# BVE-Reborn/rend3

Hardware: NVIDIA H100
Metric: culled objects/s (fused frustum cull + object-uniform bake) (higher is better)
Workload: dtype f32

## Files before the change

rend3_b200/csrc/r3_cull_bake.cu:

```cuda
#include <cstdlib>

#include "r3_common.cuh"
#include "r3_scan.cuh"

namespace {

constexpr int CB_THREADS = 256;
constexpr int CB_WARPS = CB_THREADS / 32;
constexpr int CB_WT = 4;
constexpr int CB_CTA_OBJECTS = CB_WARPS * CB_WT * 32;
constexpr int CP_THREADS = 1024;
constexpr int CP_OBJECTS = CP_THREADS * 32;
constexpr int CP_CTAS_PER_TILE = CP_OBJECTS / CB_CTA_OBJECTS;

struct CullBakeParams {
    float view[16];
    float view_proj[16];
    float frustum[5][4];
    uint32_t object_count;
};

__device__ __forceinline__ uint32_t affine_w_bits(uint32_t j) { return j == 3 ? 0x3f800000u : 0u; }

__global__ void __launch_bounds__(256) split_objects_kernel(const float4* __restrict__ objects, uint32_t n, float* __restrict__ rows_xyz, float* __restrict__ rows_w,
                                                            float4* __restrict__ spheres, uint32_t* __restrict__ enabled_bits, uint32_t* __restrict__ affine_bits) {
    const int lane = threadIdx.x & 31, k = lane & 7, g = lane >> 3;
    const uint32_t wtile = (blockIdx.x * blockDim.x + threadIdx.x) >> 5, base = wtile * 32u;
    if (base >= n) return;
    uint32_t bits = 0, abits = 0;
#pragma unroll
    for (int it = 0; it < 8; ++it) {
        const uint32_t obj = base + it * 4 + g;
        float4 r = make_float4(0.f, 0.f, 0.f, 0.f);
        if (obj < n) {
            r = __ldcs(&objects[(size_t)obj * 8 + k]);
            if (k < 4) {
                float* xyz = rows_xyz + (size_t)obj * 12 + k;
                xyz[0] = r.x; xyz[4] = r.y; xyz[8] = r.z;
                rows_w[(size_t)obj * 4 + k] = r.w;
            } else if (k == 4) spheres[obj] = r;
        }
        const uint32_t b = __ballot_sync(0xFFFFFFFFu, k == 7 && obj < n && __float_as_uint(r.y) != 0u);
        bits |= (((b >> 7) & 1u) | (((b >> 15) & 1u) << 1) | (((b >> 23) & 1u) << 2) | (((b >> 31) & 1u) << 3)) << (it * 4);
        const uint32_t a = __ballot_sync(0xFFFFFFFFu, k < 4 && obj < n && __float_as_uint(r.w) == affine_w_bits(k));
#pragma unroll
        for (int q = 0; q < 4; ++q) abits |= (((a >> (8 * q)) & 0xFu) == 0xFu ? 1u : 0u) << (it * 4 + q);
    }
    if (lane == 0) { enabled_bits[wtile] = bits; affine_bits[wtile] = abits; }
}
__global__ void __launch_bounds__(256) split_slots_kernel(const float4* __restrict__ objects, const uint32_t* __restrict__ slots, uint32_t n_updates, uint32_t n_slots,
                                                          float* __restrict__ rows_xyz, float* __restrict__ rows_w, float4* __restrict__ spheres,
                                                          uint32_t* __restrict__ enabled_bits, uint32_t* __restrict__ affine_bits) {
    const uint32_t i = (blockIdx.x * blockDim.x + threadIdx.x) >> 3, k = threadIdx.x & 7;
    const uint32_t s = i < n_updates ? slots[i] : n_slots;
    const bool ok = s < n_slots;
    float4 r = make_float4(0.f, 0.f, 0.f, 0.f);
    if (ok) {
        r = objects[(size_t)s * 8 + k];
        if (k < 4) {
            float* xyz = rows_xyz + (size_t)s * 12 + k;
            xyz[0] = r.x; xyz[4] = r.y; xyz[8] = r.z;
            rows_w[(size_t)s * 4 + k] = r.w;
        } else if (k == 4) spheres[s] = r;
    }
    const uint32_t a = __ballot_sync(0xFFFFFFFFu, ok && k < 4 && __float_as_uint(r.w) == affine_w_bits(k));
    if (ok && k == 7) {
        const uint32_t bit = 1u << (s & 31u);
        if (__float_as_uint(r.y) != 0u) atomicOr(&enabled_bits[s >> 5], bit);
        else atomicAnd(&enabled_bits[s >> 5], ~bit);
        if (((a >> (threadIdx.x & 24u)) & 0xFu) == 0xFu) atomicOr(&affine_bits[s >> 5], bit);
        else atomicAnd(&affine_bits[s >> 5], ~bit);
    }
}

template <bool BAKE, bool CULL, bool LIVE>
__global__ void __launch_bounds__(CB_THREADS)
cull_bake_kernel(const float4* __restrict__ rows_xyz, const float* __restrict__ rows_w, const uint32_t* __restrict__ affine_bits, const float4* __restrict__ spheres,
                 const uint32_t* __restrict__ enabled_bits, const uint32_t* __restrict__ live_bits, float4* __restrict__ matrices, uint32_t* __restrict__ words,
                 uint32_t* __restrict__ cta_counts, const __grid_constant__ CullBakeParams p) {
    __shared__ uint32_t s_count[CB_WARPS];
    __shared__ float4 s_rows[BAKE ? CB_WARPS : 1][96];
    const int lane = threadIdx.x & 31, warp = threadIdx.x >> 5;
    const int col = lane & 3, sub = lane >> 2;
    uint32_t count = 0;
#pragma unroll 2
    for (int wt = 0; wt < CB_WT; ++wt) {
        const uint32_t wtile = (blockIdx.x * CB_WARPS + warp) * CB_WT + wt;
        const uint32_t base = wtile * 32u;
        if (base >= p.object_count) break;
        float4 t[3];
        float4 sp = make_float4(0.f, 0.f, 0.f, 0.f);
        uint32_t enabled = 0u, affine = 0u;
        if (BAKE) {
#pragma unroll
            for (int q = 0; q < 3; ++q) {
                const uint32_t e = q * 32 + lane;
                t[q] = base + e / 3u < p.object_count ? __ldcs(&rows_xyz[(size_t)base * 3 + e]) : make_float4(0.f, 0.f, 0.f, 0.f);
            }
        }
        if (CULL && base + lane < p.object_count) sp = __ldcs(&spheres[base + lane]);
        if (BAKE || (CULL && !LIVE)) enabled = __ldg(&enabled_bits[wtile]);
        if (BAKE) affine = __ldg(&affine_bits[wtile]);
        if (BAKE) {
            float4* tile = s_rows[warp];
            __syncwarp();
#pragma unroll
            for (int q = 0; q < 3; ++q) tile[q * 32 + lane] = t[q];
            __syncwarp();
            const float* tf = reinterpret_cast<const float*>(tile);
#pragma unroll
            for (int it = 0; it < 4; ++it) {
                const uint32_t slot = it * 8 + sub, obj = base + slot;
                if (obj < p.object_count && ((enabled >> slot) & 1u)) {
                    const float* c = tf + slot * 12 + col;
                    const float w = ((affine >> slot) & 1u) ? (col == 3 ? 1.0f : 0.0f) : __ldcs(&rows_w[(size_t)obj * 4 + col]);
                    float4* dst = &matrices[(size_t)obj * 8 + col];
                    __stcs(dst, mat_vec_rn(p.view, c[0], c[4], c[8], w));
                    __stcs(dst + 4, mat_vec_rn(p.view_proj, c[0], c[4], c[8], w));
                }
            }
        }
        if (CULL) {
            const uint32_t live = LIVE ? __ldg(&live_bits[wtile]) : enabled;
            const float neg_radius = -sp.w;
            bool inside = true;
#pragma unroll
            for (int pl = 0; pl < 5; ++pl) {
                const float d = add_rn(add_rn(add_rn(mul_rn(p.frustum[pl][0], sp.x), mul_rn(p.frustum[pl][1], sp.y)), mul_rn(p.frustum[pl][2], sp.z)), p.frustum[pl][3]);
                inside = inside && (d >= neg_radius);
            }
            const uint32_t word = __ballot_sync(0xFFFFFFFFu, base + lane < p.object_count && ((live >> lane) & 1u) && inside);
            if (lane == 0) words[wtile] = word;
            count += __popc(word);
        }
    }
    if (CULL) {
        if (lane == 0) s_count[warp] = count;
        __syncthreads();
        if (threadIdx.x == 0) {
            uint32_t t = 0;
#pragma unroll
            for (int w = 0; w < CB_WARPS; ++w) t += s_count[w];
            cta_counts[blockIdx.x] = t;
        }
    }
}

constexpr uint32_t EX_HEADER_WORDS = 256;
constexpr uint32_t EX_SLOTS = R3_EXCHANGE_SLOTS;
struct ExchangeParams { uint32_t* peers[R3_MAX_EXCHANGE_RANKS]; uint32_t n_ranks, word_offset, words_per_rank, flag_offset, epoch; uint32_t* done; };

__device__ __forceinline__ void st_release_sys(uint32_t* p, uint32_t v) { asm volatile("st.release.sys.global.u32 [%0], %1;" ::"l"(p), "r"(v) : "memory"); }
__device__ __forceinline__ uint32_t ld_acquire_sys(const uint32_t* p) { uint32_t v; asm volatile("ld.acquire.sys.global.u32 %0, [%1];" : "=r"(v) : "l"(p) : "memory"); return v; }

__global__ void __launch_bounds__(CP_THREADS)
compact_visible_kernel(const uint32_t* __restrict__ words, const uint32_t* __restrict__ cta_counts, uint32_t n_words, uint32_t n_cta_counts,
                       uint32_t* __restrict__ visible, uint32_t* __restrict__ visible_count, const __grid_constant__ ExchangeParams ex) {
    __shared__ uint32_t s_warp[CP_THREADS / 32 + 1];
    const uint32_t tile_base = block_sum_u32<CP_THREADS>(cta_counts, min(blockIdx.x * CP_CTAS_PER_TILE, n_cta_counts), s_warp);
    const uint32_t wi = blockIdx.x * CP_THREADS + threadIdx.x;
    const uint32_t word = wi < n_words ? __ldg(&words[wi]) : 0u;
    if (ex.n_ranks && wi < ex.words_per_rank) {
// ... 403 lines not shown
```

rend3_b200/csrc/r3_raster.cu:

```cuda
#include "r3_common.cuh"
#include "r3_scan.cuh"
#include "r3_texture.cuh"

namespace {

constexpr int RS_THREADS = 256;
constexpr float GUARD = 64.0f;
constexpr int SMALL_AREA = 64;
constexpr int MEDIUM_MAX = 32;
constexpr int COOP_MAX_LANES = 33;
constexpr int BAND_ROWS = 16;
constexpr uint32_t LARGE_CAP = 1u << 22;
constexpr uint32_t BAND_CAP = 1u << 24;
constexpr uint32_t BAND_SKIP = 0xFFFFFFFFu;
constexpr int MODE_COLOUR = 0;
constexpr int MODE_DEPTH = 1;
constexpr int MODE_BLEND = 2;
constexpr int MODE_MSAA = 4;
constexpr int MODE_ALPHA = 8;

struct SubTri { int32_t x[3], y[3]; float z[3]; uint32_t rec; };
constexpr uint32_t REC_ALPHA_TESTED = 0x80000000u;
static_assert(sizeof(SubTri) == 40, "SubTri");

struct RasterParams {
    const r3_batch_data* batches; const r3_region* regions; const uint32_t* header;
    const r3_indirect_call* calls; const uint32_t* indices; uint64_t index_elems;
    const unsigned long long* tri_prefix;
    const r3_object* objects; uint32_t n_slots;
    const r3_object_matrices* matrices; uint32_t matrices_cap;
    const uint32_t* mesh; uint64_t mesh_words;
    const r3_material* materials; uint32_t n_materials;
    TexTable tt;
    float ox, oy, vw, vh; int32_t x0, y0, x1, y1; uint32_t pitch; int positive_visible;
    uint32_t samples;
    unsigned long long* vis; uint32_t pass_bit;
    uint32_t* depth_bits;
    r3_tri_record* records;
    SubTri* large; uint2* bands; uint32_t* counters;
    uint32_t* frag_heads; uint4* frag_nodes; uint32_t frag_cap;
    unsigned long long key_lo, key_hi;
    unsigned long long* stats;
};

__device__ __forceinline__ uint32_t mesh_word(const RasterParams& p, uint64_t i) { return i < p.mesh_words ? __ldg(&p.mesh[i]) : 0u; }

__device__ __forceinline__ float plane_dist(int plane, const float4 v) {
    switch (plane) {
        case 0: return v.z;
        case 1: return sub_rn(v.w, v.z);
        case 2: return add_rn(v.x, mul_rn(GUARD, v.w));
        case 3: return sub_rn(mul_rn(GUARD, v.w), v.x);
        case 4: return add_rn(v.y, mul_rn(GUARD, v.w));
        default: return sub_rn(mul_rn(GUARD, v.w), v.y);
    }
}
__device__ __forceinline__ float4 clip_lerp(const float4 in, const float4 out, float din, float dout) {
    const float t = div_rn(din, sub_rn(din, dout));
    return make_float4(add_rn(in.x, mul_rn(t, sub_rn(out.x, in.x))), add_rn(in.y, mul_rn(t, sub_rn(out.y, in.y))),
                       add_rn(in.z, mul_rn(t, sub_rn(out.z, in.z))), add_rn(in.w, mul_rn(t, sub_rn(out.w, in.w))));
}
__device__ __noinline__ int clip_polygon(float4* poly, int n) {
    for (int plane = 0; plane < 6 && n >= 3; ++plane) {
        bool any_out = false;
        for (int i = 0; i < n; ++i) any_out |= plane_dist(plane, poly[i]) < 0.0f;
        if (!any_out) continue;
        float4 outp[12];
        int m = 0;
        for (int i = 0; i < n; ++i) {
            const float4 a = poly[i], b = poly[(i + 1) % n];
            const float da = plane_dist(plane, a), db = plane_dist(plane, b);
            if (da >= 0.0f) {
                outp[m++] = a;
                if (db < 0.0f) outp[m++] = clip_lerp(a, b, da, db);
            } else if (db >= 0.0f) {
                outp[m++] = clip_lerp(b, a, db, da);
            }
        }
        n = m;
        for (int i = 0; i < n; ++i) poly[i] = outp[i];
    }
    return n >= 3 ? n : 0;
}

constexpr int FITS32_REACH = 11585;
template <typename T>
struct EdgeSetupT {
    T e0, e1, e2;
    T sx0, sx1, sx2;
    T sy0, sy1, sy2;
    int b0, b1, b2;
    float inv_area;
};
__device__ __forceinline__ float to_float_rn(long long v) { return __ll2float_rn(v); }
__device__ __forceinline__ float to_float_rn(int v) { return __int2float_rn(v); }
__device__ __forceinline__ long long edge_fn(int ax, int ay, int bx, int by, long long px, long long py) {
    return (long long)(bx - ax) * (py - ay) - (long long)(by - ay) * (px - ax);
}
__device__ __forceinline__ int not_top_left(int ax, int ay, int bx, int by) {
    const int dx = bx - ax, dy = by - ay;
    return ((dy < 0) || (dy == 0 && dx > 0)) ? 0 : 1;
}
__device__ __forceinline__ bool fits32(const SubTri& s, int px0, int py0, int px1, int py1) {
    const int ox = px0 * 256 + 128, oy = py0 * 256 + 128;
    int reach = max((px1 - px0) * 256 + 128, (py1 - py0) * 256 + 128);
#pragma unroll
    for (int k = 0; k < 3; ++k) reach = max(reach, max(abs(s.x[k] - ox), abs(s.y[k] - oy)));
    return reach <= FITS32_REACH && abs(px0) < (1 << 20) && abs(py0) < (1 << 20);
}
template <typename T>
__device__ __forceinline__ EdgeSetupT<T> make_edges(const SubTri& s, int px, int py) {
    EdgeSetupT<T> e;
    e.b0 = not_top_left(s.x[1], s.y[1], s.x[2], s.y[2]);
    e.b1 = not_top_left(s.x[2], s.y[2], s.x[0], s.y[0]);
    e.b2 = not_top_left(s.x[0], s.y[0], s.x[1], s.y[1]);
    const int ox = px * 256 + 128, oy = py * 256 + 128;
    const T x0 = (T)s.x[0] - ox, y0 = (T)s.y[0] - oy, x1 = (T)s.x[1] - ox, y1 = (T)s.y[1] - oy, x2 = (T)s.x[2] - ox, y2 = (T)s.y[2] - oy;
    e.e0 = (x2 - x1) * (-y1) - (y2 - y1) * (-x1) - e.b0;
    e.e1 = (x0 - x2) * (-y2) - (y0 - y2) * (-x2) - e.b1;
    e.e2 = (x1 - x0) * (-y0) - (y1 - y0) * (-x0) - e.b2;
    e.sx0 = -(y2 - y1) * 256; e.sy0 = (x2 - x1) * 256;
    e.sx1 = -(y0 - y2) * 256; e.sy1 = (x0 - x2) * 256;
    e.sx2 = -(y1 - y0) * 256; e.sy2 = (x1 - x0) * 256;
    const T area = (x1 - x0) * (y2 - y0) - (y1 - y0) * (x2 - x0);
    e.inv_area = div_rn(1.0f, to_float_rn(area));
    return e;
}
template <typename T>
__device__ __forceinline__ float sample_depth(const SubTri& s, const EdgeSetupT<T>& e, T e0, T e1, T e2) {
    const float la = mul_rn(to_float_rn((T)(e0 + e.b0)), e.inv_area), lb = mul_rn(to_float_rn((T)(e1 + e.b1)), e.inv_area),
                lc = mul_rn(to_float_rn((T)(e2 + e.b2)), e.inv_area);
    const float z = add_rn(add_rn(mul_rn(la, s.z[0]), mul_rn(lb, s.z[1])), mul_rn(lc, s.z[2]));
    return fminf(fmaxf(z, 0.0f), 1.0f);
}
template <int MODE>
__device__ __forceinline__ uint32_t write_sample(const RasterParams& p, int px, int py, uint32_t k, float z, uint32_t rec) {
    const size_t pi = (size_t)py * p.pitch + px;
    if ((MODE & 3) == MODE_DEPTH) {
        atomicMax(&p.depth_bits[pi], __float_as_uint(z));
    } else if ((MODE & 3) == MODE_COLOUR) {
        const unsigned long long key = ((unsigned long long)__float_as_uint(z) << 32) | ((unsigned long long)p.pass_bit << 31) | (rec & ~REC_ALPHA_TESTED);
        atomicMax(&p.vis[pi * p.samples + k], key);
    } else {
        const size_t si = pi * p.samples + k;
        if (__float_as_uint(z) >= (uint32_t)(p.vis[si] >> 32)) {
            const uint32_t node = atomicAdd(&p.counters[3], 1u);
            if (node < p.frag_cap) {
                const uint32_t next = atomicExch(&p.frag_heads[si], node + 1u);
                p.frag_nodes[node] = make_uint4(rec & ~REC_ALPHA_TESTED, __float_as_uint(z), next, 0u);
            }
        }
        return 0u;
    }
    return 1u;
}

__device__ __constant__ int c_sample_dx[4] = {-32, 96, -96, 32};
__device__ __constant__ int c_sample_dy[4] = {-96, -32, 32, 96};

template <int MODE>
__device__ __noinline__ bool cutout_discards(const RasterParams& p, uint32_t rec, int px, int py) {
    const r3_tri_record* tp = p.records + ((rec & ~REC_ALPHA_TESTED) - 1u);
    const float4 q0 = reinterpret_cast<const float4*>(tp)[0], q1 = reinterpret_cast<const float4*>(tp)[1], q2 = reinterpret_cast<const float4*>(tp)[2];
    const uint4 q3 = reinterpret_cast<const uint4*>(tp)[3];
    const float p0[3] = {q0.x, q0.y, q0.z}, p1[3] = {q0.w, q1.x, q1.y}, p2[3] = {q1.z, q1.w, q2.x};
    const uint32_t oid = __float_as_uint(q2.y);
    const uint32_t vid[3] = {__float_as_uint(q2.z), __float_as_uint(q2.w), q3.x};
    const r3_object* obj = &p.objects[oid];
    const r3_material* m = &p.materials[obj->material_index < p.n_materials ? obj->material_index : 0u];
    const uint32_t flags = m->flags;
    float alpha = 1.0f;
    if (flags & R3_MAT_ALBEDO_ACTIVE) {
        const float hw = p.vw * 0.5f, hh = p.vh * 0.5f;
        float b[3][3];
#pragma unroll
        for (int k = 0; k < 3; ++k) {
            const float fx = ((float)px - p.ox) + (k == 1 ? 1.5f : 0.5f), fy = ((float)py - p.oy) + (k == 2 ? 1.5f : 0.5f);
            const float nx = fx / hw - 1.0f, ny = 1.0f - fy / hh;
            const float b0 = ((p1[1] * p2[2] - p1[2] * p2[1]) * nx + (p1[2] * p2[0] - p1[0] * p2[2]) * ny) + (p1[0] * p2[1] - p1[1] * p2[0]);
            const float b1 = ((p2[1] * p0[2] - p2[2] * p0[1]) * nx + (p2[2] * p0[0] - p2[0] * p0[2]) * ny) + (p2[0] * p0[1] - p2[1] * p0[0]);
            const float b2 = ((p0[1] * p1[2] - p0[2] * p1[1]) * nx + (p0[2] * p1[0] - p0[0] * p1[2]) * ny) + (p0[0] * p1[1] - p0[1] * p1[0]);
            const float sum = (b0 + b1) + b2;
            b[k][0] = b0 / sum; b[k][1] = b1 / sum; b[k][2] = b2 / sum;
        }
        const uint32_t albedo_tex = m->textures[R3_TEX_ALBEDO];
        if (albedo_tex) {
            float uv[3][2] = {{0.f, 0.f}, {0.f, 0.f}, {0.f, 0.f}};
            const uint32_t uv_off = obj->attr_offset[3];
            if (uv_off != R3_ATTR_ABSENT) {
#pragma unroll
                for (int k = 0; k < 3; ++k) {
                    const uint64_t w = (uint64_t)(uv_off >> 2) + (uint64_t)vid[k] * 2u;
                    uv[k][0] = __uint_as_float(mesh_word(p, w)); uv[k][1] = __uint_as_float(mesh_word(p, w + 1));
                }
            }
            float co[3][2];
#pragma unroll
            for (int k = 0; k < 3; ++k) {
                const float u = (b[k][0] * uv[0][0] + b[k][1] * uv[1][0]) + b[k][2] * uv[2][0];
                const float v = (b[k][0] * uv[0][1] + b[k][1] * uv[1][1]) + b[k][2] * uv[2][1];
                if ((MODE & 3) == MODE_DEPTH) { co[k][0] = u; co[k][1] = v; }
                else {
                    co[k][0] = (m->uv_transform0[0][0] * u + m->uv_transform0[1][0] * v) + m->uv_transform0[2][0];
                    co[k][1] = (m->uv_transform0[0][1] * u + m->uv_transform0[1][1] * v) + m->uv_transform0[2][1];
                }
            }
            TexCoords tc;
            tc.u = co[0][0]; tc.v = co[0][1];
            tc.dudx = co[1][0] - co[0][0]; tc.dvdx = co[1][1] - co[0][1];
            if ((MODE & 3) == MODE_DEPTH) { tc.dudy = tc.dudx; tc.dvdy = tc.dvdx; }
            else { tc.dudy = co[2][0] - co[0][0]; tc.dvdy = co[2][1] - co[0][1]; }
            alpha = texture_sample_grad(p.tt, albedo_tex, (MODE & 3) != MODE_DEPTH && (flags & R3_MAT_NEAREST), tc).w;
        }
        if (flags & R3_MAT_ALBEDO_BLEND) {
            float va[3] = {1.0f, 1.0f, 1.0f};
            const uint32_t col_off = obj->attr_offset[5];
            if (col_off != R3_ATTR_ABSENT) {
#pragma unroll
                for (int k = 0; k < 3; ++k) va[k] = (float)(mesh_word(p, (uint64_t)(col_off >> 2) + vid[k]) >> 24) / 255.0f;
            }
            alpha *= (b[0][0] * va[0] + b[0][1] * va[1]) + b[0][2] * va[2];
        }
    }
    return alpha * m->albedo[3] < m->alpha_cutout;
}

template <int MODE, typename T>
__device__ __forceinline__ void emit_pixel(const RasterParams& p, const SubTri& s, const EdgeSetupT<T>& e, int px, int py, T c0, T c1, T c2, uint32_t& frags) {
    if (!(MODE & MODE_MSAA)) {
        if ((c0 | c1 | c2) >= 0) {
            if ((MODE & MODE_ALPHA) && (s.rec & REC_ALPHA_TESTED) && cutout_discards<MODE>(p, s.rec, px, py)) return;
            frags += write_sample<MODE>(p, px, py, 0u, sample_depth<T>(s, e, c0, c1, c2), s.rec);
        }
        return;
    }
    bool tested = !(MODE & MODE_ALPHA) || !(s.rec & REC_ALPHA_TESTED);
#pragma unroll
    for (int k = 0; k < 4; ++k) {
        const T a0 = c0 + (e.sx0 >> 8) * c_sample_dx[k] + (e.sy0 >> 8) * c_sample_dy[k];
        const T a1 = c1 + (e.sx1 >> 8) * c_sample_dx[k] + (e.sy1 >> 8) * c_sample_dy[k];
        const T a2 = c2 + (e.sx2 >> 8) * c_sample_dx[k] + (e.sy2 >> 8) * c_sample_dy[k];
        if ((a0 | a1 | a2) >= 0) {
            if (!tested) {
                if (cutout_discards<MODE>(p, s.rec, px, py)) return;
                tested = true;
            }
            frags += write_sample<MODE>(p, px, py, (uint32_t)k, sample_depth<T>(s, e, a0, a1, a2), s.rec);
        }
    }
}

__device__ __forceinline__ void pixel_bounds(const RasterParams& p, const SubTri& s, int& px0, int& py0, int& px1, int& py1) {
    const int minx = min(s.x[0], min(s.x[1], s.x[2])), maxx = max(s.x[0], max(s.x[1], s.x[2]));
    const int miny = min(s.y[0], min(s.y[1], s.y[2])), maxy = max(s.y[0], max(s.y[1], s.y[2]));
    if (p.samples == 1u) {
        px0 = max((minx - 128 + 255) >> 8, p.x0); px1 = min((maxx - 128) >> 8, p.x1 - 1);
        py0 = max((miny - 128 + 255) >> 8, p.y0); py1 = min((maxy - 128) >> 8, p.y1 - 1);
    } else {
        px0 = max(minx >> 8, p.x0); px1 = min(maxx >> 8, p.x1 - 1);
        py0 = max(miny >> 8, p.y0); py1 = min(maxy >> 8, p.y1 - 1);
    }
}

template <int MODE, typename T>
__device__ __forceinline__ void raster_inline_t(const RasterParams& p, const SubTri& s, int px0, int py0, int px1, int py1, uint32_t& frags) {
    const EdgeSetupT<T> e = make_edges<T>(s, px0, py0);
    T r0 = e.e0, r1 = e.e1, r2 = e.e2;
    for (int py = py0; py <= py1; ++py) {
        T c0 = r0, c1 = r1, c2 = r2;
        for (int px = px0; px <= px1; ++px) {
            emit_pixel<MODE, T>(p, s, e, px, py, c0, c1, c2, frags);
            c0 += e.sx0; c1 += e.sx1; c2 += e.sx2;
        }
        r0 += e.sy0; r1 += e.sy1; r2 += e.sy2;
    }
}
template <int MODE>
__device__ __forceinline__ void raster_inline(const RasterParams& p, const SubTri& s, int px0, int py0, int px1, int py1, uint32_t& frags) {
    if (fits32(s, px0, py0, px1, py1)) raster_inline_t<MODE, int>(p, s, px0, py0, px1, py1, frags);
    else raster_inline_t<MODE, long long>(p, s, px0, py0, px1, py1, frags);
}

template <int MODE>
__device__ bool process_subtriangle(const RasterParams& p, const float4 a, const float4 b, const float4 c, uint32_t rec, uint32_t& frags, SubTri* defer,
                                    bool* deferred) {
    const float4 v[3] = {a, b, c};
    int sx[3], sy[3];
    float sz[3];
    const float hw = mul_rn(p.vw, 0.5f), hh = mul_rn(p.vh, 0.5f);
#pragma unroll
    for (int k = 0; k < 3; ++k) {
        if (!(v[k].w > 0.0f)) return false;
        const bool unit_w = v[k].w == 1.0f;
        const float nx = unit_w ? v[k].x : div_rn(v[k].x, v[k].w), ny = unit_w ? v[k].y : div_rn(v[k].y, v[k].w), nz = unit_w ? v[k].z : div_rn(v[k].z, v[k].w);
        const float fx = add_rn(p.ox, mul_rn(add_rn(nx, 1.0f), hw)), fy = add_rn(p.oy, mul_rn(sub_rn(1.0f, ny), hh));
        const float qx = rintf(mul_rn(fx, 256.0f)), qy = rintf(mul_rn(fy, 256.0f));
        if (!(fabsf(qx) < 1.0e9f) || !(fabsf(qy) < 1.0e9f)) return false;
        sx[k] = (int)qx; sy[k] = (int)qy; sz[k] = nz;
    }
    const long long area = (long long)(sx[1] - sx[0]) * (sy[2] - sy[0]) - (long long)(sx[2] - sx[0]) * (sy[1] - sy[0]);
    if (area == 0) return false;
    const bool visible = p.positive_visible ? (area < 0) : (area > 0);
    if (!visible) return false;
    SubTri s;
    if (area > 0) {
#pragma unroll
        for (int k = 0; k < 3; ++k) { s.x[k] = sx[k]; s.y[k] = sy[k]; s.z[k] = sz[k]; }
    } else {
        s.x[0] = sx[0]; s.y[0] = sy[0]; s.z[0] = sz[0]; s.x[1] = sx[2]; s.y[1] = sy[2]; s.z[1] = sz[2]; s.x[2] = sx[1]; s.y[2] = sy[1]; s.z[2] = sz[1];
    }
    s.rec = rec;
    int px0, py0, px1, py1;
    pixel_bounds(p, s, px0, py0, px1, py1);
    if (px0 > px1 || py0 > py1) return true;
    const int w = px1 - px0 + 1, h = py1 - py0 + 1;
    bool inline_raster = (w * h <= SMALL_AREA);
    if (!inline_raster && defer && w <= MEDIUM_MAX && h <= MEDIUM_MAX) {
        *defer = s;
        *deferred = true;
        return true;
    }
    if (!inline_raster) {
        const uint32_t nb = (uint32_t)((py1 / BAND_ROWS) - (py0 / BAND_ROWS) + 1);
        const uint32_t li = atomicAdd(&p.counters[0], 1u);
        uint32_t bi = 0;
        bool queued = li < LARGE_CAP;
        if (queued) {
            bi = atomicAdd(&p.counters[1], nb);
            queued = bi + nb <= BAND_CAP;
            if (!queued) for (uint32_t k = bi; k < BAND_CAP; ++k) p.bands[k] = make_uint2(BAND_SKIP, 0u);
        }
        if (queued) {
            p.large[li] = s;
            for (uint32_t k = 0; k < nb; ++k) p.bands[bi + k] = make_uint2(li, (uint32_t)(py0 / BAND_ROWS) + k);
            return true;
        }
        if (defer) {
            *defer = s;
            *deferred = true;
            return true;
        }
        inline_raster = true;
    }
    raster_inline<MODE>(p, s, px0, py0, px1, py1, frags);
    return true;
}

template <int MODE, typename T>
__device__ __forceinline__ void raster_cooperative_t(const RasterParams& p, const SubTri& s, int lane, int px0, int py0, int px1, int py1, uint32_t& frags) {
    const int w = px1 - px0 + 1;
    const int lw = w <= 8 ? 8 : (w <= 16 ? 16 : 32), lh = 32 / lw, lx = lane % lw, ly = lane / lw;
    const EdgeSetupT<T> e = make_edges<T>(s, px0, py0);
    for (int py = py0 + ly; py <= py1; py += lh) {
        const T dy = py - py0;
        T c0 = e.e0 + dy * e.sy0 + (T)lx * e.sx0, c1 = e.e1 + dy * e.sy1 + (T)lx * e.sx1, c2 = e.e2 + dy * e.sy2 + (T)lx * e.sx2;
        for (int px = px0 + lx; px <= px1; px += lw) {
            emit_pixel<MODE, T>(p, s, e, px, py, c0, c1, c2, frags);
            c0 += lw * e.sx0; c1 += lw * e.sx1; c2 += lw * e.sx2;
        }
    }
}
template <int MODE>
__device__ __forceinline__ void raster_cooperative(const RasterParams& p, const SubTri& s, int lane, uint32_t& frags) {
    int px0, py0, px1, py1;
    pixel_bounds(p, s, px0, py0, px1, py1);
    if (fits32(s, px0, py0, px1, py1)) raster_cooperative_t<MODE, int>(p, s, lane, px0, py0, px1, py1, frags);
    else raster_cooperative_t<MODE, long long>(p, s, lane, px0, py0, px1, py1, frags);
}

template <int MODE>
__device__ void setup_listed_triangle(const RasterParams& p, unsigned long long i, uint32_t n_regions, uint32_t& frags, uint32_t& set_up, SubTri* defer, bool* deferred) {
    uint32_t lo = 0, hi = n_regions;
    while (hi - lo > 1) {
        const uint32_t mid = (lo + hi) >> 1;
        if (p.tri_prefix[mid] <= i) lo = mid; else hi = mid;
    }
    const uint32_t r = lo;
    const uint32_t t = (uint32_t)(i - p.tri_prefix[r]);
    const uint64_t e = (uint64_t)p.calls[r].base_index + (uint64_t)t * 3u;
    if (e + 2 >= p.index_elems) return;
    const uint32_t k0 = p.indices[e], k1 = p.indices[e + 1], k2 = p.indices[e + 2];
    if (k0 == R3_INVALID_VERTEX || k1 == R3_INVALID_VERTEX || k2 == R3_INVALID_VERTEX) return;
    const r3_batch_data* batch = &p.batches[p.regions[r].job_index];
    const uint32_t oid = batch->object_culling_information[k0 >> 24].object_id;
    if (oid >= p.n_slots || oid >= p.matrices_cap) return;
    const r3_object* obj = &p.objects[oid];
    if (obj->enabled == 0u) return;
    bool alpha_tested = false;
    if (p.regions[r].material_key == 1ull) {
        const r3_material* m = &p.materials[obj->material_index < p.n_materials ? obj->material_index : 0u];
        alpha_tested = (m->flags & R3_MAT_ALBEDO_ACTIVE) && (m->textures[R3_TEX_ALBEDO] != 0u || ((m->flags & R3_MAT_ALBEDO_BLEND) && obj->attr_offset[5] != R3_ATTR_ABSENT));
        if (!alpha_tested && m->albedo[3] < m->alpha_cutout) return;
        if (!(MODE & MODE_ALPHA) || !p.records) alpha_tested = false;
    }
    const uint32_t pos_off = obj->attr_offset[0] >> 2;
    float mvp[16];
    {
        const float4* m4 = reinterpret_cast<const float4*>(p.matrices[oid].model_view_proj);
#pragma unroll
        for (int q = 0; q < 4; ++q) { const float4 c4 = __ldg(&m4[q]); mvp[4 * q] = c4.x; mvp[4 * q + 1] = c4.y; mvp[4 * q + 2] = c4.z; mvp[4 * q + 3] = c4.w; }
    }
    const uint32_t vid[3] = {k0 & 0xFFFFFFu, k1 & 0xFFFFFFu, k2 & 0xFFFFFFu};
    float4 clip[3];
#pragma unroll
    for (int k = 0; k < 3; ++k) {
        const uint64_t f = (uint64_t)pos_off + (uint64_t)vid[k] * 3u;
        if (f + 2u < p.mesh_words) clip[k] = mat_point_rn(mvp, __uint_as_float(__ldg(&p.mesh[f])), __uint_as_float(__ldg(&p.mesh[f + 1])), __uint_as_float(__ldg(&p.mesh[f + 2])));
        else clip[k] = mat_point_rn(mvp, __uint_as_float(mesh_word(p, f)), __uint_as_float(mesh_word(p, f + 1)), __uint_as_float(mesh_word(p, f + 2)));
    }
    bool ox0 = true, ox1 = true, oy0 = true, oy1 = true, oz0 = true, oz1 = true, need_clip = false, nan = false;
#pragma unroll
    for (int k = 0; k < 3; ++k) {
        const float4 v = clip[k];
        ox0 &= v.x < -v.w; ox1 &= v.x > v.w; oy0 &= v.y < -v.w; oy1 &= v.y > v.w; oz0 &= v.z < 0.0f; oz1 &= v.z > v.w;
#pragma unroll
        for (int pl = 0; pl < 6; ++pl) need_clip |= plane_dist(pl, v) < 0.0f;
        nan |= !(v.w == v.w);
    }
    if (nan || ox0 || ox1 || oy0 || oy1 || oz0 || oz1) return;
    const uint32_t rec = (uint32_t)(i + 1) | (alpha_tested ? REC_ALPHA_TESTED : 0u);
    const auto store_record = [&]() {
        r3_tri_record tr;
#pragma unroll
        for (int k = 0; k < 3; ++k) { tr.xyw[k][0] = clip[k].x; tr.xyw[k][1] = clip[k].y; tr.xyw[k][2] = clip[k].w; tr.vid[k] = vid[k]; }
        tr.object_id = oid; tr._pad[0] = tr._pad[1] = tr._pad[2] = 0u;
        float4* dst = reinterpret_cast<float4*>(&p.records[i]);
        const float4* src = reinterpret_cast<const float4*>(&tr);
        dst[0] = src[0]; dst[1] = src[1]; dst[2] = src[2]; dst[3] = src[3];
    };
    if (alpha_tested) store_record();
    bool any = false;
    if (!need_clip) {
        any = process_subtriangle<MODE>(p, clip[0], clip[1], clip[2], rec, frags, defer, deferred);
    } else {
        float4 poly[12];
        poly[0] = clip[0]; poly[1] = clip[1]; poly[2] = clip[2];
        const int n = clip_polygon(poly, 3);
        for (int q = 1; q + 1 < n; ++q) any |= process_subtriangle<MODE>(p, poly[0], poly[q], poly[q + 1], rec, frags, nullptr, nullptr);
    }
    if (any) {
        set_up++;
        if ((MODE & 3) != MODE_DEPTH && !alpha_tested) store_record();
    }
}

template <int MODE>
__global__ void __launch_bounds__(RS_THREADS, MODE == MODE_DEPTH ? 4 : 1) raster_setup_kernel(const __grid_constant__ RasterParams p) {
    const uint32_t n_regions = p.header[2];
    const unsigned long long total = p.tri_prefix[n_regions];
    const int lane = threadIdx.x & 31;
    uint32_t frags = 0, set_up = 0;
    for (;;) {
        uint32_t tile = 0;
        if (lane == 0) tile = atomicAdd(&p.counters[4], 1u);
        tile = __shfl_sync(0xFFFFFFFFu, tile, 0);
        const unsigned long long base = (unsigned long long)tile * 32ull;
        if (base >= total) break;
        const unsigned long long i = base + lane;
        SubTri med;
        bool has_med = false;
        if (i < total) setup_listed_triangle<MODE>(p, i, n_regions, frags, set_up, &med, &has_med);
        if (MODE & MODE_ALPHA) __syncwarp();
        uint32_t m = __ballot_sync(0xFFFFFFFFu, has_med);
        if (__popc(m) >= COOP_MAX_LANES) {
            if (has_med) {
                int px0, py0, px1, py1;
                pixel_bounds(p, med, px0, py0, px1, py1);
                raster_inline<MODE>(p, med, px0, py0, px1, py1, frags);
            }
            m = 0;
        }
        while (m) {
            const int src = __ffs(m) - 1;
            m &= m - 1;
            SubTri s;
#pragma unroll
            for (int k = 0; k < 3; ++k) {
                s.x[k] = __shfl_sync(0xFFFFFFFFu, med.x[k], src); s.y[k] = __shfl_sync(0xFFFFFFFFu, med.y[k], src); s.z[k] = __shfl_sync(0xFFFFFFFFu, med.z[k], src);
            }
            s.rec = __shfl_sync(0xFFFFFFFFu, med.rec, src);
            raster_cooperative<MODE>(p, s, lane, frags);
        }
    }
    frags = warp_reduce(frags);
    set_up = warp_reduce(set_up);
    if (lane == 0 && p.stats) {
        if (set_up) atomicAdd(&p.stats[0], (unsigned long long)set_up);
        if (frags) atomicAdd(&p.stats[1], (unsigned long long)frags);
    }
}

template <int MODE>
__global__ void __launch_bounds__(RS_THREADS) raster_band_kernel(const __grid_constant__ RasterParams p) {
    const int lane = threadIdx.x & 31;
    uint32_t n_bands = p.counters[1];
    if (n_bands > BAND_CAP) n_bands = BAND_CAP;
    uint32_t frags = 0;
    for (;;) {
        uint32_t item = 0;
        if (lane == 0) item = atomicAdd(&p.counters[2], 1u);
        item = __shfl_sync(0xFFFFFFFFu, item, 0);
        if (item >= n_bands) break;
        const uint2 it = p.bands[item];
        if (it.x >= LARGE_CAP) continue;
        const SubTri s = p.large[it.x];
        int px0, py0, px1, py1;
        pixel_bounds(p, s, px0, py0, px1, py1);
        const int by0 = max(py0, (int)it.y * BAND_ROWS), by1 = min(py1, (int)it.y * BAND_ROWS + BAND_ROWS - 1);
        if (by0 > by1) continue;
        const EdgeSetupT<long long> e = make_edges<long long>(s, px0, by0);
        const int rows = by1 - by0 + 1;
        for (int bx = px0; bx <= px1; bx += 32) {
            const long long dx = bx - px0, wx = min(31, px1 - bx), hy = rows - 1;
            const long long k0 = p.samples == 1u ? 0 : (llabs(e.sx0) + llabs(e.sy0)) / 2, k1 = p.samples == 1u ? 0 : (llabs(e.sx1) + llabs(e.sy1)) / 2,
                            k2 = p.samples == 1u ? 0 : (llabs(e.sx2) + llabs(e.sy2)) / 2;
            const long long m0 = k0 + e.e0 + dx * e.sx0 + (e.sx0 > 0 ? wx * e.sx0 : 0) + (e.sy0 > 0 ? hy * e.sy0 : 0);
            const long long m1 = k1 + e.e1 + dx * e.sx1 + (e.sx1 > 0 ? wx * e.sx1 : 0) + (e.sy1 > 0 ? hy * e.sy1 : 0);
            const long long m2 = k2 + e.e2 + dx * e.sx2 + (e.sx2 > 0 ? wx * e.sx2 : 0) + (e.sy2 > 0 ? hy * e.sy2 : 0);
            if ((m0 | m1 | m2) < 0) continue;
            const int px = bx + lane;
            long long c0 = e.e0 + (dx + lane) * e.sx0, c1 = e.e1 + (dx + lane) * e.sx1, c2 = e.e2 + (dx + lane) * e.sx2;
            for (int py = by0; py <= by1; ++py) {
                if (px <= px1) emit_pixel<MODE, long long>(p, s, e, px, py, c0, c1, c2, frags);
                c0 += e.sy0; c1 += e.sy1; c2 += e.sy2;
            }
        }
    }
    frags = warp_reduce(frags);
    if (lane == 0 && frags && p.stats) atomicAdd(&p.stats[1], (unsigned long long)frags);
}

constexpr int RP_THREADS = 1024;
__global__ void __launch_bounds__(RP_THREADS) region_prefix_kernel(const r3_region* __restrict__ regions, const r3_indirect_call* __restrict__ calls,
                                                                   const uint32_t* __restrict__ header, unsigned long long* __restrict__ prefix,
                                                                   unsigned long long key_lo, unsigned long long key_hi) {
    __shared__ unsigned long long s_warp[RP_THREADS / 32 + 1];
    const uint32_t n_regions = header[2];
    const unsigned long long total = block_scan_excl_chunked<RP_THREADS>(
        n_regions, s_warp,
        [&](uint32_t r) {
            return regions[r].material_key >= key_lo && regions[r].material_key <= key_hi ? (unsigned long long)(calls[r].vertex_count / 3u) : 0ull;
        },
        [&](uint32_t r, unsigned long long e) { prefix[r] = e; });
    if (threadIdx.x == 0) prefix[n_regions] = total;
}

}

template <void (*K)(const RasterParams)>
static int resident_grid(const r3_ctx* c) {
    static int per_sm = 0;
    if (!per_sm && (cudaOccupancyMaxActiveBlocksPerMultiprocessor(&per_sm, K, RS_THREADS, 0) != cudaSuccess || per_sm < 1)) { cudaGetLastError(); per_sm = 1; }
    return c->sm_count * per_sm;
}
struct DrawSource { const r3_jobs* jobs; const r3_indirect_call* calls; const uint32_t* indices; uint64_t index_elems; };

static bool draw_source_for(r3_camera* cam, int jobs_idx, int partition, DrawSource* ds) {
    if (!cam->index_buffer.created || jobs_idx < 0) return false;
    const r3_jobs* j = &cam->jobs[jobs_idx];
    if (!j->valid || (!j->device_built && j->n_regions == 0)) return false;
    const r3_iobuf& ib = cam->index_buffer; const r3_iobuf& db = cam->draw_call_buffer;
    if (j->n_regions > db.capacity_elements / 2) return false;
    ds->jobs = j;
    ds->indices = (const uint32_t*)ib.d + (partition ? ib.in_off() : ib.out_off());
    ds->index_elems = ib.capacity_elements / 2;
    ds->calls = (const r3_indirect_call*)db.d + (partition ? db.in_off() : db.out_off());
    return true;
}

static int ensure_raster_scratch(r3_ctx* c) {
    const uint64_t need = 64 + (uint64_t)LARGE_CAP * sizeof(SubTri) + (uint64_t)BAND_CAP * sizeof(uint2);
    return r3_reserve(c, &c->d_scratch, &c->scratch_cap, need, 1, false, false);
}

static int run_raster(r3_ctx* c, r3_camera* cam, const DrawSource& ds, int mode, int pass, float ox, float oy, float vw, float vh,
                      int x0, int y0, int x1, int y1, uint32_t pitch) {
    const bool depth_only = mode == MODE_DEPTH;
    const r3_jobs* j = ds.jobs;
    R3_TRY(ensure_raster_scratch(c));
    uint32_t* counters = (uint32_t*)c->d_scratch;
    SubTri* large = (SubTri*)((uint8_t*)c->d_scratch + 64);
    uint2* bands = (uint2*)((uint8_t*)large + (size_t)LARGE_CAP * sizeof(SubTri));
    R3_CUDA(c, cudaMemsetAsync(counters, 0, 64, c->stream));
    R3_TRY(r3_reserve_t(c, &cam->d_block_sums, &cam->block_sums_cap, (uint64_t)j->n_regions + 2));
    const unsigned long long key_lo = mode == MODE_BLEND ? 2ull : 0ull, key_hi = mode == MODE_BLEND ? 2ull : 1ull;
    region_prefix_kernel<<<1, RP_THREADS, 0, c->stream>>>(j->d_regions, ds.calls, j->d_header, cam->d_block_sums, key_lo, key_hi);
    R3_CHECK_LAUNCH(c, "region_prefix_kernel");

    RasterParams p;
    p.batches = j->d_batches; p.regions = j->d_regions; p.header = j->d_header;
    p.calls = ds.calls; p.indices = ds.indices; p.index_elems = ds.index_elems; p.tri_prefix = cam->d_block_sums;
    p.objects = c->d_objects; p.n_slots = c->n_slots; p.matrices = cam->d_matrices; p.matrices_cap = cam->matrices_cap;
    p.mesh = c->d_mesh; p.mesh_words = c->mesh_words; p.materials = c->d_materials; p.n_materials = c->n_materials;
    p.ox = ox; p.oy = oy; p.vw = vw; p.vh = vh; p.x0 = x0; p.y0 = y0; p.x1 = x1; p.y1 = y1; p.pitch = pitch;
    p.positive_visible = (cam->header.flags & R3_PCU_POSITIVE_AREA_VISIBLE) ? 1 : 0;
    p.samples = depth_only ? 1u : c->samples;
    p.vis = c->d_vis; p.pass_bit = (uint32_t)(pass & 1); p.depth_bits = (uint32_t*)c->d_atlas;
    p.frag_heads = c->d_frag_heads; p.frag_nodes = c->d_frag_nodes; p.frag_cap = (uint32_t)c->frag_nodes_cap; p.key_lo = key_lo; p.key_hi = key_hi;
    p.large = large; p.bands = bands; p.counters = counters; p.stats = mode == MODE_COLOUR ? c->d_stats : nullptr;
    p.tt.tex = c->d_tex_descs; p.tt.n_tex = c->n_textures; p.tt.texels = c->d_texels; p.tt.clamp_to_edge = 0u;
    p.records = nullptr;
    if (depth_only && c->any_frag_alpha) {
        R3_TRY(r3_reserve_t(c, &c->d_tris[3], &c->tris_cap[3], (uint64_t)j->total_invocations + 1));
        p.records = c->d_tris[3];
    }
    if (!depth_only) {
        const uint64_t max_tris = (uint64_t)j->total_invocations;
        if (max_tris >= (1ull << 31)) return r3_fail(c, R3_E_INVALID, "more than 2^31 triangles in one pass");
        R3_TRY(r3_reserve_t(c, &c->d_tris[pass], &c->tris_cap[pass], max_tris + 1));
        c->n_tris[pass] = max_tris;
        p.records = c->d_tris[pass];
    }
    const int variant = mode | ((mode != MODE_DEPTH && c->samples == 4u) ? MODE_MSAA : 0) | ((c->any_frag_alpha && mode != MODE_BLEND) ? MODE_ALPHA : 0);
#define R3_RASTER_ONE(KERNEL, M) KERNEL<M><<<resident_grid<KERNEL<M>>(c), RS_THREADS, 0, c->stream>>>(p)
#define R3_RASTER_LAUNCH(KERNEL)                                                                                          \
    switch (variant) {                                                                                                    \
        case MODE_DEPTH: R3_RASTER_ONE(KERNEL, MODE_DEPTH); break;                                                        \
        case MODE_COLOUR: R3_RASTER_ONE(KERNEL, MODE_COLOUR); break;                                                      \
        case MODE_BLEND: R3_RASTER_ONE(KERNEL, MODE_BLEND); break;                                                        \
        case MODE_COLOUR | MODE_MSAA: R3_RASTER_ONE(KERNEL, MODE_COLOUR | MODE_MSAA); break;                              \
        case MODE_BLEND | MODE_MSAA: R3_RASTER_ONE(KERNEL, MODE_BLEND | MODE_MSAA); break;                                \
        case MODE_DEPTH | MODE_ALPHA: R3_RASTER_ONE(KERNEL, MODE_DEPTH | MODE_ALPHA); break;                              \
        case MODE_COLOUR | MODE_ALPHA: R3_RASTER_ONE(KERNEL, MODE_COLOUR | MODE_ALPHA); break;                            \
        default: R3_RASTER_ONE(KERNEL, MODE_COLOUR | MODE_MSAA | MODE_ALPHA); break;                                      \
    }
    r3_stage_begin(c, depth_only ? R3_STAGE_RASTER_SETUP_DEPTH : R3_STAGE_RASTER_SETUP_COLOUR);
    R3_RASTER_LAUNCH(raster_setup_kernel)
    r3_stage_end(c);
    R3_CHECK_LAUNCH(c, "raster_setup_kernel");
    r3_stage_begin(c, R3_STAGE_RASTER_BANDS);
    R3_RASTER_LAUNCH(raster_band_kernel)
    r3_stage_end(c);
    R3_CHECK_LAUNCH(c, "raster_band_kernel");
#undef R3_RASTER_LAUNCH
#undef R3_RASTER_ONE
// ... 54 lines not shown
```

Measured before the change: 14.07 billion.

## Add warp-cooperative span walk for medium depth-only triangles and defer clipping

In depth-only rasterization, medium triangles that fit 32-bit edge math are handed to a new warp-wide scanline walker. It packs the per-triangle edge setup into shared memory, spreads rows across lanes, computes each row's covered span, then spreads pixels across lanes for atomicMax depth writes. Triangles that need clipping are parked in shared memory and clipped in a separate noinline routine after the walk, which keeps register pressure in the main path low and reduces divergence. Separately, the cull/bake kernel's per-warp object tile count drops from 4 to 1. The measured metric is cull/bake throughput, so only that knob change likely matters for it.

```diff
diff --git a/rend3_b200/csrc/r3_cull_bake.cu b/rend3_b200/csrc/r3_cull_bake.cu
--- a/rend3_b200/csrc/r3_cull_bake.cu
+++ b/rend3_b200/csrc/r3_cull_bake.cu
@@ -7,7 +7,7 @@
 
 constexpr int CB_THREADS = 256;
 constexpr int CB_WARPS = CB_THREADS / 32;
-constexpr int CB_WT = 4;
+constexpr int CB_WT = 1;
 constexpr int CB_CTA_OBJECTS = CB_WARPS * CB_WT * 32;
 constexpr int CP_THREADS = 1024;
 constexpr int CP_OBJECTS = CP_THREADS * 32;
diff --git a/rend3_b200/csrc/r3_raster.cu b/rend3_b200/csrc/r3_raster.cu
--- a/rend3_b200/csrc/r3_raster.cu
+++ b/rend3_b200/csrc/r3_raster.cu
@@ -127,11 +127,14 @@
     return e;
 }
 template <typename T>
+__device__ __forceinline__ float plane_depth(float inv_area, float z0, float z1, float z2, T w0, T w1, T w2) {
+    const float la = mul_rn(to_float_rn(w0), inv_area), lb = mul_rn(to_float_rn(w1), inv_area), lc = mul_rn(to_float_rn(w2), inv_area);
+    const float z = add_rn(add_rn(mul_rn(la, z0), mul_rn(lb, z1)), mul_rn(lc, z2));
+    return fminf(fmaxf(z, 0.0f), 1.0f);
+}
+template <typename T>
 __device__ __forceinline__ float sample_depth(const SubTri& s, const EdgeSetupT<T>& e, T e0, T e1, T e2) {
-    const float la = mul_rn(to_float_rn((T)(e0 + e.b0)), e.inv_area), lb = mul_rn(to_float_rn((T)(e1 + e.b1)), e.inv_area),
-                lc = mul_rn(to_float_rn((T)(e2 + e.b2)), e.inv_area);
-    const float z = add_rn(add_rn(mul_rn(la, s.z[0]), mul_rn(lb, s.z[1])), mul_rn(lc, s.z[2]));
-    return fminf(fmaxf(z, 0.0f), 1.0f);
+    return plane_depth<T>(e.inv_area, s.z[0], s.z[1], s.z[2], (T)(e0 + e.b0), (T)(e1 + e.b1), (T)(e2 + e.b2));
 }
 template <int MODE>
 __device__ __forceinline__ uint32_t write_sample(const RasterParams& p, int px, int py, uint32_t k, float z, uint32_t rec) {
@@ -281,9 +284,14 @@
     else raster_inline_t<MODE, long long>(p, s, px0, py0, px1, py1, frags);
 }
 
+constexpr int DEFER_NONE = 0;
+constexpr int DEFER_COOP = 1;
+constexpr int DEFER_WALK = 2;
+constexpr int DEFER_CLIP = 3;
+
 template <int MODE>
 __device__ bool process_subtriangle(const RasterParams& p, const float4 a, const float4 b, const float4 c, uint32_t rec, uint32_t& frags, SubTri* defer,
-                                    bool* deferred) {
+                                    int* deferred) {
     const float4 v[3] = {a, b, c};
     int sx[3], sy[3];
     float sz[3];
@@ -314,10 +322,15 @@
     pixel_bounds(p, s, px0, py0, px1, py1);
     if (px0 > px1 || py0 > py1) return true;
     const int w = px1 - px0 + 1, h = py1 - py0 + 1;
+    if ((MODE & 3) == MODE_DEPTH && defer && w * h > SMALL_AREA && w <= MEDIUM_MAX && h <= MEDIUM_MAX && fits32(s, px0, py0, px1, py1)) {
+        *defer = s;
+        *deferred = DEFER_WALK;
+        return true;
+    }
     bool inline_raster = (w * h <= SMALL_AREA);
     if (!inline_raster && defer && w <= MEDIUM_MAX && h <= MEDIUM_MAX) {
         *defer = s;
-        *deferred = true;
+        *deferred = DEFER_COOP;
         return true;
     }
     if (!inline_raster) {
@@ -337,7 +350,7 @@
         }
         if (defer) {
             *defer = s;
-            *deferred = true;
+            *deferred = DEFER_COOP;
             return true;
         }
         inline_raster = true;
@@ -368,8 +381,114 @@
     else raster_cooperative_t<MODE, long long>(p, s, lane, px0, py0, px1, py1, frags);
 }
 
-template <int MODE>
-__device__ void setup_listed_triangle(const RasterParams& p, unsigned long long i, uint32_t n_regions, uint32_t& frags, uint32_t& set_up, SubTri* defer, bool* deferred) {
+struct DepthWalkWarp {
+    int4 edge[32];
+    int4 step_y[32];
+    int4 step_x[32];
+    float4 depth[32];
+    uint4 misc[32];
+    int4 span[32];
+    int4 span_at[32];
+    float4 clip[32][3];
+    uint32_t clip_rec[32];
+};
+
+__device__ __forceinline__ int item_at(bool has, int start, int base, int lane) {
+    const uint32_t before = __popc(__ballot_sync(0xFFFFFFFFu, has && start < base));
+    const uint32_t starts = __reduce_or_sync(0xFFFFFFFFu, (has && start >= base && start - base < 32) ? 1u << (start - base) : 0u);
+    return (int)(before + __popc(starts & ((2u << lane) - 1u))) - 1;
+}
+
+__device__ __forceinline__ void edge_span(int r, int s, int w, int& lo, int& hi) {
+    if (s > 0) {
+        int x = (int)fminf(fmaxf(ceilf(__fdividef(-(float)r, (float)s)), 0.0f), (float)w);
+        while (x > 0 && r + (x - 1) * s >= 0) --x;
+        while (x < w && r + x * s < 0) ++x;
+        lo = max(lo, x);
+    } else if (s < 0) {
+        int x = (int)fminf(fmaxf(floorf(__fdividef((float)r, -(float)s)), -1.0f), (float)(w - 1));
+        while (x < w - 1 && r + (x + 1) * s >= 0) ++x;
+        while (x >= 0 && r + x * s < 0) --x;
+        hi = min(hi, x);
+    } else if (r < 0) {
+        hi = -1;
+    }
+}
+
+template <int MODE>
+__device__ __forceinline__ void depth_walk(const RasterParams& p, DepthWalkWarp& w, bool has, const SubTri& s, int lane) {
+    const uint32_t entries = __ballot_sync(0xFFFFFFFFu, has);
+    if (!entries) return;
+    const int rank = __popc(entries & ((1u << lane) - 1u));
+    int px0 = 0, py0 = 0, px1 = 0, py1 = 0;
+    if (has) pixel_bounds(p, s, px0, py0, px1, py1);
+    const int rows = has ? py1 - py0 + 1 : 0;
+    const int rows_end = warp_scan_incl(rows), rows_start = rows_end - rows;
+    const int n_rows = __shfl_sync(0xFFFFFFFFu, rows_end, 31);
+    if (has) {
+        const EdgeSetupT<int> e = make_edges<int>(s, px0, py0);
+        w.edge[rank] = make_int4(e.e0, e.e1, e.e2, rows_start);
+        w.step_y[rank] = make_int4(e.sy0, e.sy1, e.sy2, px0);
+        w.step_x[rank] = make_int4(e.sx0, e.sx1, e.sx2, py0);
+        w.depth[rank] = make_float4(e.inv_area, s.z[0], s.z[1], s.z[2]);
+        w.misc[rank] = make_uint4((uint32_t)(e.b0 | e.b1 << 1 | e.b2 << 2), s.rec, (uint32_t)(px1 - px0 + 1), 0u);
+    }
+    __syncwarp();
+    for (int rb = 0; rb < n_rows; rb += 32) {
+        const int t = item_at(has, rows_start, rb, lane);
+        int len = 0, lo = 0;
+        int4 c = make_int4(0, 0, 0, 0), at = make_int4(0, 0, 0, 0);
+        if (rb + lane < n_rows) {
+            const int4 ed = w.edge[t], sy = w.step_y[t], sx = w.step_x[t];
+            const int bw = (int)w.misc[t].z, y = rb + lane - ed.w;
+            const int r0 = ed.x + y * sy.x, r1 = ed.y + y * sy.y, r2 = ed.z + y * sy.z;
+            int hi = bw - 1;
+            edge_span(r0, sx.x, bw, lo, hi);
+            edge_span(r1, sx.y, bw, lo, hi);
+            edge_span(r2, sx.z, bw, lo, hi);
+            len = max(hi - lo + 1, 0);
+            c = make_int4(r0 + lo * sx.x, r1 + lo * sx.y, r2 + lo * sx.z, 0);
+            at = make_int4(sy.w + lo, sx.w + y, t, 0);
+        }
+        const int px_end = warp_scan_incl(len), px_start = px_end - len;
+        const int n_px = __shfl_sync(0xFFFFFFFFu, px_end, 31);
+        const uint32_t spans = __ballot_sync(0xFFFFFFFFu, len > 0);
+        __syncwarp();
+        if (len > 0) {
+            const int q = __popc(spans & ((1u << lane) - 1u));
+            w.span[q] = make_int4(c.x, c.y, c.z, px_start);
+            w.span_at[q] = at;
+        }
+        __syncwarp();
+        for (int pb = 0; pb < n_px; pb += 32) {
+            const int q = item_at(len > 0, px_start, pb, lane);
+            if (pb + lane >= n_px) continue;
+            const int4 sp = w.span[q], sa = w.span_at[q];
+            const int d = pb + lane - sp.w, x = sa.x + d;
+            const uint4 mi = w.misc[sa.z];
+            if ((MODE & MODE_ALPHA) && (mi.y & REC_ALPHA_TESTED) && cutout_discards<MODE>(p, mi.y, x, sa.y)) continue;
+            const int4 sx = w.step_x[sa.z];
+            const float4 dz = w.depth[sa.z];
+            const float z = plane_depth<int>(dz.x, dz.y, dz.z, dz.w, sp.x + d * sx.x + (int)(mi.x & 1u), sp.y + d * sx.y + (int)((mi.x >> 1) & 1u),
+                                             sp.z + d * sx.z + (int)(mi.x >> 2));
+            atomicMax(&p.depth_bits[(size_t)sa.y * p.pitch + x], __float_as_uint(z));
+        }
+    }
+}
+
+template <int MODE>
+__device__ __noinline__ uint32_t raster_clipped(const RasterParams& p, const float4* clip, uint32_t rec) {
+    float4 poly[12];
+    poly[0] = clip[0]; poly[1] = clip[1]; poly[2] = clip[2];
+    const int n = clip_polygon(poly, 3);
+    uint32_t frags = 0;
+    for (int q = 1; q + 1 < n; ++q) process_subtriangle<MODE>(p, poly[0], poly[q], poly[q + 1], rec, frags, nullptr, nullptr);
+    return frags;
+}
+
+template <int MODE>
+__device__ void setup_listed_triangle(const RasterParams& p, unsigned long long i, uint32_t n_regions, uint32_t& frags, uint32_t& set_up, SubTri* defer,
+                                      int* deferred, float4* clip_slot, uint32_t* clip_rec) {
     uint32_t lo = 0, hi = n_regions;
     while (hi - lo > 1) {
         const uint32_t mid = (lo + hi) >> 1;
@@ -432,6 +551,11 @@
     bool any = false;
     if (!need_clip) {
         any = process_subtriangle<MODE>(p, clip[0], clip[1], clip[2], rec, frags, defer, deferred);
+    } else if ((MODE & 3) == MODE_DEPTH && clip_slot) {
+        clip_slot[0] = clip[0]; clip_slot[1] = clip[1]; clip_slot[2] = clip[2];
+        *clip_rec = rec;
+        *deferred = DEFER_CLIP;
+        return;
     } else {
         float4 poly[12];
         poly[0] = clip[0]; poly[1] = clip[1]; poly[2] = clip[2];
@@ -444,11 +568,15 @@
     }
 }
 
-template <int MODE>
-__global__ void __launch_bounds__(RS_THREADS, MODE == MODE_DEPTH ? 4 : 1) raster_setup_kernel(const __grid_constant__ RasterParams p) {
+constexpr int SETUP_DEPTH_CTAS = 4;
+template <int MODE>
+__global__ void __launch_bounds__(RS_THREADS, MODE == MODE_DEPTH ? SETUP_DEPTH_CTAS : 1) raster_setup_kernel(const __grid_constant__ RasterParams p) {
     const uint32_t n_regions = p.header[2];
     const unsigned long long total = p.tri_prefix[n_regions];
     const int lane = threadIdx.x & 31;
+    constexpr bool depth = (MODE & 3) == MODE_DEPTH;
+    __shared__ DepthWalkWarp s_walk[depth ? RS_THREADS / 32 : 1];
+    DepthWalkWarp& walk = s_walk[depth ? threadIdx.x >> 5 : 0];
     uint32_t frags = 0, set_up = 0;
     for (;;) {
         uint32_t tile = 0;
@@ -458,9 +586,12 @@
         if (base >= total) break;
         const unsigned long long i = base + lane;
         SubTri med;
-        bool has_med = false;
-        if (i < total) setup_listed_triangle<MODE>(p, i, n_regions, frags, set_up, &med, &has_med);
-        if (MODE & MODE_ALPHA) __syncwarp();
+        int deferred = DEFER_NONE;
+        if (i < total)
+            setup_listed_triangle<MODE>(p, i, n_regions, frags, set_up, &med, &deferred, depth ? walk.clip[lane] : nullptr, depth ? &walk.clip_rec[lane] : nullptr);
+        if ((MODE & MODE_ALPHA) || depth) __syncwarp();
+        if (depth) depth_walk<MODE>(p, walk, deferred == DEFER_WALK, med, lane);
+        const bool has_med = deferred == DEFER_COOP;
         uint32_t m = __ballot_sync(0xFFFFFFFFu, has_med);
         if (__popc(m) >= COOP_MAX_LANES) {
             if (has_med) {
@@ -481,6 +612,7 @@
             s.rec = __shfl_sync(0xFFFFFFFFu, med.rec, src);
             raster_cooperative<MODE>(p, s, lane, frags);
         }
+        if (depth && deferred == DEFER_CLIP) frags += raster_clipped<MODE>(p, walk.clip[lane], walk.clip_rec[lane]);
     }
     frags = warp_reduce(frags);
     set_up = warp_reduce(set_up);
```

New measurement: 14.36 billion, median of 6. 2.1% higher.
